# Banksylel/Restrictive-Hierarchical-Semantic-Segmentation

Measured on AMD Instinct MI355X. Metric: train images/sec (620x620, hier-HRNet-W48), higher is better.
Workload: dtype f32 (fp16x2 split on fp16 MFMA, 22-bit operands, fp32 accumulate; exact-fp32 MFMA on the small problems); 1 GPU; HRNet-W48 hierarchical (class_tree_tl.json), 620x620, batch 4 per GPU, train_epoch batch body (fwd L passes, prediction prep + metrics, CE+Dice+consistency, bwd, grad all-reduce, AdamW, metric vectors, one D2H readback of loss+metrics); global_batch=4, parallelism=dp1, launch=launch tape replay, rccl_ranks=1, level_passes=batched (one launch per layer for all L passes)

## Files before the change

restrictive-hierarchical-semantic-segmentation_amd/csrc/conv_sp.h:

```cpp
#pragma once
#include <type_traits>

typedef __bf16 bf16x8 __attribute__((ext_vector_type(8)));
typedef __bf16 bf16x2 __attribute__((ext_vector_type(2)));
typedef unsigned u32x4 __attribute__((ext_vector_type(4)));
typedef unsigned u32x2 __attribute__((ext_vector_type(2)));

__device__ __forceinline__ unsigned sp_pack_trunc(float lo, float hi) {
  return __builtin_amdgcn_perm(__float_as_uint(hi), __float_as_uint(lo), 0x07060302u);
}
__device__ __forceinline__ unsigned sp_pack_rne(float lo, float hi) {
  const bf16x2 v = {(__bf16)lo, (__bf16)hi};
  return __builtin_bit_cast(unsigned, v);
}
__device__ __forceinline__ float sp_trunc(float x) { return __uint_as_float(__float_as_uint(x) & 0xFFFF0000u); }

constexpr int sp_np(int ns) { return ns == 4 ? 2 : ns; }
constexpr int sp_products(int ns) { return ns == 1 ? 1 : ns == 3 ? 6 : 3; }
typedef _Float16 f16x8 __attribute__((ext_vector_type(8)));
typedef _Float16 f16x2 __attribute__((ext_vector_type(2)));

__device__ __forceinline__ void sp_pow2_scale(const float* absmax, float& scale, float& inv) {
  scale = inv = 1.f;
  if (!absmax) return;
// ... 1006 lines not shown
      u32x2 pc[sp_np(NS)];
      sp_split4<NS>(rp[i], pc, xscale);
      int f = tid + 256 * i;
      if (f >= PG) f -= 256;
      const int pix = f / (CS * 4), rem = f - pix * (CS * 4);
      const int c = rem >> 2, q = rem & 3;
      const int o = c * L::CHUNK + pix * 32 + ((q ^ (2 * ((pix >> 3) & 1))) << 3);
#pragma unroll
      for (int s = 0; s < sp_np(NS); ++s) *reinterpret_cast<u32x2*>(lpatch + s * L::PPIECE + o) = pc[s];
    }
  };

  unsigned wrow[W_LOADS];
  int wst[W_LOADS];
#pragma unroll
  for (int i = 0; i < W_LOADS; ++i) {
    int f = tid + 256 * i;
    if (f >= WG) f -= 256;
    const int n = f >> 3, unit = (f >> 2) & 1, gq = f & 3;
    wrow[i] = ((unsigned)n * (unsigned)(p.T * p.K) + 4u * gq) * 4u;
    wst[i] = n * 64 + lds_slot(n, gq) * 16 + unit * 8;
  }
  const bool wunit1 = (tid >> 2) & 1;
  f32x4 rwt[2][W_LOADS];
  constexpr int W16 = NS == 4 ? L::WSTAGE / 16 : 0;
  static_assert(W16 <= 256 * W_LOADS, "a pre-split slab fits the register set of an fp32 one");
  const bool img = NS == 4 && p.wimg != nullptr;
  const __amdgpu_buffer_rsrc_t rwi = make_rsrc(reinterpret_cast<const float*>(p.wimg), (size_t)ntn * nks * NSLAB * L::WSTAGE);
  auto w_load = [&](int n0, int ks, int slab, int set) {
    if (img) {
      const unsigned base = (unsigned)(((n0 / BN) * nks + ks) * NSLAB + slab) * (unsigned)L::WSTAGE;
#pragma unroll
      for (int i = 0; i < W_LOADS; ++i) {
        const int f = tid + 256 * i;
        rwt[set][i] = buf_load4(rwi, f < W16 ? base + (unsigned)f * 16u : HRSEG_BUF_OOB, 0);
      }
      return;
    }
    const int uA = 2 * slab, uB = 2 * slab + 1;
    const int tA = uA / CS, cA = uA - tA * CS, tB = uB / CS, cB = uB - tB * CS;
    const unsigned col0 = (unsigned)(n0 * p.T * p.K + ks * CS * 16) * 4u;
    const unsigned sA = col0 + (unsigned)(tA * p.K + cA * 16) * 4u;
    const unsigned sB = (uB < NU) ? col0 + (unsigned)(tB * p.K + cB * 16) * 4u : HRSEG_BUF_OOB;
    const unsigned so = wunit1 ? sB : sA;
#pragma unroll
    for (int i = 0; i < W_LOADS; ++i) {
      const unsigned off = (so == HRSEG_BUF_OOB) ? HRSEG_BUF_OOB : wrow[i] + so;
      rwt[set][i] = buf_load4(rw, off, 0);
    }
  };
  auto w_store = [&](int wboff, int set) {
    unsigned char* base = lw + wboff;
    if (img) {
#pragma unroll
      for (int i = 0; i < W_LOADS; ++i) {
        const int f = tid + 256 * i;
        if (f < W16) *reinterpret_cast<f32x4*>(base + f * 16) = rwt[set][i];
      }
      return;
    }
#pragma unroll
    for (int i = 0; i < W_LOADS; ++i) {
      u32x2 pc[sp_np(NS)];
      sp_split4<NS>(rwt[set][i], pc, p.wscale);
#pragma unroll
      for (int s = 0; s < sp_np(NS); ++s) *reinterpret_cast<u32x2*>(base + s * L::WPIECE + wst[i]) = pc[s];
    }
  };

  const int foff = r16 * 64 + lds_slot(r16, g) * 16;
  const int prow0 = (wave * RPW) * PW + r16;
  const int pbase = prow0 * 32;

  auto read_frags = [&](int slab, int wboff, bf16x8 (&xf)[RPW][sp_np(NS)], bf16x8 (&wf)[WTN][sp_np(NS)]) {
    const int uA = 2 * slab, uB = 2 * slab + 1;
    const int tA = uA / CS, cA = uA - tA * CS;
    const int tB = (uB < NU) ? uB / CS : 0, cB = (uB < NU) ? uB - tB * CS : 0;
    const int dA = (FLIP ? 2 - tA / 3 : tA / 3) * PW + (FLIP ? 2 - tA % 3 : tA % 3);
    const int dB = (FLIP ? 2 - tB / 3 : tB / 3) * PW + (FLIP ? 2 - tB % 3 : tB % 3);
#pragma unroll
    for (int m = 0; m < RPW; ++m) {
      const int pa = prow0 + m * PW + dA, pb = prow0 + m * PW + dB;
      const int oa = cA * L::CHUNK + pbase + (m * PW + dA) * 32 + ((g ^ (2 * ((pa >> 3) & 1))) << 3);
      const int ob = cB * L::CHUNK + pbase + (m * PW + dB) * 32 + ((g ^ (2 * ((pb >> 3) & 1))) << 3);
#pragma unroll
      for (int q = 0; q < sp_np(NS); ++q) {
        const u32x2 lo = *reinterpret_cast<const u32x2*>(lpatch + q * L::PPIECE + oa);
        u32x2 hi = u32x2{0u, 0u};
        if (uB < NU) hi = *reinterpret_cast<const u32x2*>(lpatch + q * L::PPIECE + ob);
        xf[m][q] = __builtin_bit_cast(bf16x8, (u32x4){lo[0], lo[1], hi[0], hi[1]});
      }
    }
    const unsigned char* base = lw + wboff;
#pragma unroll
    for (int n = 0; n < WTN; ++n)
#pragma unroll
      for (int q = 0; q < sp_np(NS); ++q) wf[n][q] = *reinterpret_cast<const bf16x8*>(base + q * L::WPIECE + n * 1024 + foff);
  };

  f32x4 acc[WTN][RPW];
  auto zero_acc = [&]() {
#pragma unroll
    for (int n = 0; n < WTN; ++n)
#pragma unroll
      for (int m = 0; m < RPW; ++m) acc[n][m] = f32x4{0.f, 0.f, 0.f, 0.f};
  };
  auto store_tile = [&](const Geom& q) {
    f32x4 add[RPW][WTN];
#pragma unroll
    for (int n = 0; n < WTN; ++n) {
      f32x4 bv = f32x4{0.f, 0.f, 0.f, 0.f};
      if (p.bias) bv = *reinterpret_cast<const f32x4*>(p.bias + q.n0 + 16 * n + 4 * g);
#pragma unroll
      for (int m = 0; m < RPW; ++m) add[m][n] = bv;
    }
    if (p.accumulate) {
#pragma unroll
      for (int m = 0; m < RPW; ++m) {
        const int oy = q.y0 + wave * RPW + m, ox = q.x0 + r16;
        if (oy >= H || ox >= W) continue;
        const float* yrow = p.y + ((size_t)(q.b * H + oy) * W + ox) * p.ldy;
#pragma unroll
        for (int n = 0; n < WTN; ++n) add[m][n] += *reinterpret_cast<const f32x4*>(yrow + q.n0 + 16 * n + 4 * g);
      }
    }
    if (p.res) {
#pragma unroll
      for (int m = 0; m < RPW; ++m) {
        const int oy = q.y0 + wave * RPW + m, ox = q.x0 + r16;
        if (oy >= H || ox >= W) continue;
        const float* rrow = p.res + ((size_t)(q.b * H + oy) * W + ox) * p.ldr;
#pragma unroll
        for (int n = 0; n < WTN; ++n) add[m][n] += *reinterpret_cast<const f32x4*>(rrow + q.n0 + 16 * n + 4 * g);
      }
    }
#pragma unroll
    for (int m = 0; m < RPW; ++m) {
      const int oy = q.y0 + wave * RPW + m, ox = q.x0 + r16;
      if (oy >= H || ox >= W) continue;
      float* yrow = p.y + ((size_t)(q.b * H + oy) * W + ox) * p.ldy;
#pragma unroll
      for (int n = 0; n < WTN; ++n) {
        f32x4 v = acc[n][m];
        if (NS == 4) v *= oscale;
        v += add[m][n];
        if (p.relu) {
#pragma unroll
          for (int e = 0; e < 4; ++e) v[e] = fmaxf(v[e], 0.f);
        }
        *reinterpret_cast<f32x4*>(yrow + q.n0 + 16 * n + 4 * g) = v;
      }
    }
  };

  bf16x8 xfr[2][RPW][sp_np(NS)], wfr[2][WTN][sp_np(NS)];
  int t = first;
  Geom cur = tile_geom(t);
  patch_load(cur, 0);
  w_load(cur.n0, 0, 0, 0);
  w_load(cur.n0, 0, 1, 1);
  patch_store();
  w_store(0, 0);
  w_store(L::WSTAGE, 1);
  w_load(cur.n0, 0, 2, 0);
  __syncthreads();
  read_frags(0, 0, xfr[0], wfr[0]);
  zero_acc();
  int wb = 0;
  for (;;) {
    bool have_next = false;
    for (int ks = 0; ks < nks; ++ks) {
      const bool last_ks = ks + 1 == nks;
      const int nt = last_ks ? t + stride : t;
      const int nks_ = last_ks ? 0 : ks + 1;
      have_next = nt < end;
      Geom nxt = cur;
      if (last_ks && have_next) nxt = tile_geom(nt);
#pragma unroll
      for (int s = 0; s < NSLAB; ++s) {
        const int wb1 = (wb == 2 * L::WSTAGE) ? 0 : wb + L::WSTAGE;
        const int wb2 = (wb1 == 2 * L::WSTAGE) ? 0 : wb1 + L::WSTAGE;
        if (s + 3 < NSLAB) w_load(cur.n0, ks, s + 3, (s + 1) & 1);
        else if (have_next) w_load(nxt.n0, nks_, s + 3 - NSLAB, (s + 1) & 1);
        if (s == NSLAB - 3 && have_next) patch_load(nxt, nks_);
        if (s + 1 < NSLAB) read_frags(s + 1, wb1, xfr[(s + 1) & 1], wfr[(s + 1) & 1]);
#pragma unroll
        for (int pr = 0; pr < sp_nprod(NS); ++pr)
#pragma unroll
          for (int n = 0; n < WTN; ++n)
#pragma unroll
            for (int m = 0; m < RPW; ++m) acc[n][m] = sp_mma_p<NS>(pr, wfr[s & 1][n], xfr[s & 1][m], acc[n][m]);
        if (s + 2 < NSLAB || have_next) w_store(wb2, s & 1);
        if (s == NSLAB - 1) {
          if (last_ks) { store_tile(cur); zero_acc(); }
          if (have_next) patch_store();
        }
        __syncthreads();
        if (s == NSLAB - 1 && have_next) read_frags(0, wb1, xfr[0], wfr[0]);
        wb = wb1;
      }
      if (last_ks) cur = nxt;
    }
    if (!have_next) break;
    t += stride;
  }
}

constexpr int sp_patch_min_waves(int ns, int wtn, int cs) { return (ns == 3 || (wtn == 6 && cs == 4)) ? 1 : 2; }
template <int NS, int TH, int WTN, int CS, int FLIP>
__global__ __launch_bounds__(256) __attribute__((amdgpu_waves_per_eu(sp_patch_min_waves(NS, WTN, CS), 2)))
void igemm_patch_sp_kernel(IgemmArgs p, int ntotal) {
  __shared__ __attribute__((aligned(16))) unsigned char lds[SpPatchLds<NS, TH, WTN, CS>::BYTES];
  const int chunk = (ntotal + gridDim.x - 1) / gridDim.x;
  const int first = blockIdx.x * chunk;
  igemm_patch_sp_body<NS, TH, WTN, CS, FLIP>(p, lds, first, 1, min(first + chunk, ntotal));
}

template <int NS, int TH, int WTN, int CS>
struct SpPatchWsLds {
  using P = SpPatchLds<NS, TH, WTN, CS>;
  static constexpr int STAT_MAXN = 1024;
  static constexpr int STAT = 2 * STAT_MAXN * 8;
  static constexpr int BYTES = 2 * P::PATCH + 3 * P::WSTAGE + STAT;
  static constexpr int NSLAB = (9 * CS + 1) / 2;
};

template <int NS, int WTN, int CS>
__device__ __forceinline__ void sp_weight_image_body(const float* __restrict__ w, unsigned char* __restrict__ img, int K,
                                                     float wscale, int blk) {
  using L = SpPatchLds<NS, 8, WTN, CS>;
  constexpr int BN = 16 * WTN, WG = BN * 8, NU = 9 * CS, NSLAB = (NU + 1) / 2;
  const int nks = K / (16 * CS);
  const int slab = blk % NSLAB;
  const int ks = (blk / NSLAB) % nks;
  const int nt = blk / (NSLAB * nks);
  unsigned char* dst = img + (size_t)blk * L::WSTAGE;
  for (int f = threadIdx.x; f < WG; f += 256) {
    const int n = f >> 3, unit = (f >> 2) & 1, gq = f & 3;
    const int u = 2 * slab + unit;
    f32x4 v = {0.f, 0.f, 0.f, 0.f};
    if (u < NU) {
      const int t = u / CS, c = u - t * CS;
      v = *reinterpret_cast<const f32x4*>(w + ((size_t)(nt * BN + n) * 9 + t) * K + ks * CS * 16 + c * 16 + 4 * gq);
    }
    u32x2 pc[sp_np(NS)];
    sp_split4<NS>(v, pc, wscale);
    const int o = n * 64 + lds_slot(n, gq) * 16 + unit * 8;
#pragma unroll
    for (int q = 0; q < sp_np(NS); ++q) *reinterpret_cast<u32x2*>(dst + q * L::WPIECE + o) = pc[q];
  }
}
struct WeightImageGroup {
  int n;
  int ns;
  int blk_end[MAXG];
  int kind[MAXG];
  int K[MAXG];
  float wscale[MAXG];
  const float* w[MAXG];
  unsigned char* img[MAXG];
};
struct WeightImageTabEntry {
  const float* w;
  unsigned char* img;
  int K, kind, ns, blk_end;
  float wscale;
  int pad;
};
#ifdef HRSEG_TU_WS
__global__ __launch_bounds__(256) void sp_weight_image_table_kernel(const WeightImageTabEntry* __restrict__ tab, int n) {
  int lo = 0, hi = n - 1;
  while (lo < hi) {
    const int mid = (lo + hi) >> 1;
    if ((int)blockIdx.x >= tab[mid].blk_end) lo = mid + 1; else hi = mid;
  }
  const WeightImageTabEntry e = tab[lo];
  const int blk = blockIdx.x - (lo ? tab[lo - 1].blk_end : 0);
  if (e.ns == 1) {
    if (e.kind == 2) sp_weight_image_body<1, 6, 3>(e.w, e.img, e.K, e.wscale, blk);
    else if (e.kind == 3) sp_weight_image_body<1, 4, 4>(e.w, e.img, e.K, e.wscale, blk);
    else sp_weight_image_body<1, 3, 3>(e.w, e.img, e.K, e.wscale, blk);
    return;
  }
  if (e.kind == 2) sp_weight_image_body<4, 6, 3>(e.w, e.img, e.K, e.wscale, blk);
  else if (e.kind == 3) sp_weight_image_body<4, 4, 4>(e.w, e.img, e.K, e.wscale, blk);
  else sp_weight_image_body<4, 3, 3>(e.w, e.img, e.K, e.wscale, blk);
}
__global__ __launch_bounds__(256) void sp_weight_image_kernel(WeightImageGroup g) {
  int gi = 0;
  while (gi + 1 < g.n && (int)blockIdx.x >= g.blk_end[gi]) ++gi;
  const int blk = blockIdx.x - (gi ? g.blk_end[gi - 1] : 0);
  const int kind = g.kind[gi];
  if (g.ns == 1) {
    if (kind == 2) sp_weight_image_body<1, 6, 3>(g.w[gi], g.img[gi], g.K[gi], g.wscale[gi], blk);
    else if (kind == 3) sp_weight_image_body<1, 4, 4>(g.w[gi], g.img[gi], g.K[gi], g.wscale[gi], blk);
    else sp_weight_image_body<1, 3, 3>(g.w[gi], g.img[gi], g.K[gi], g.wscale[gi], blk);
    return;
  }
  if (kind == 2) sp_weight_image_body<4, 6, 3>(g.w[gi], g.img[gi], g.K[gi], g.wscale[gi], blk);
  else if (kind == 3) sp_weight_image_body<4, 4, 4>(g.w[gi], g.img[gi], g.K[gi], g.wscale[gi], blk);
  else sp_weight_image_body<4, 3, 3>(g.w[gi], g.img[gi], g.K[gi], g.wscale[gi], blk);
}
#endif

__device__ __forceinline__ float sp_row16_sum(float v) {
  v += __builtin_bit_cast(float, __builtin_amdgcn_update_dpp(0, __builtin_bit_cast(int, v), 0x111, 0xf, 0xf, true));
  v += __builtin_bit_cast(float, __builtin_amdgcn_update_dpp(0, __builtin_bit_cast(int, v), 0x112, 0xf, 0xf, true));
  v += __builtin_bit_cast(float, __builtin_amdgcn_update_dpp(0, __builtin_bit_cast(int, v), 0x114, 0xf, 0xf, true));
  v += __builtin_bit_cast(float, __builtin_amdgcn_update_dpp(0, __builtin_bit_cast(int, v), 0x118, 0xf, 0xf, true));
  return v;
}

__device__ __forceinline__ void sp_wait_vm(f32x4& r, int n) {
  switch (n) {
#define HRSEG_VM(N) case N: asm volatile("s_waitcnt vmcnt(" #N ")" : "+v"(r)); break;
    HRSEG_VM(0) HRSEG_VM(1) HRSEG_VM(2) HRSEG_VM(3) HRSEG_VM(4) HRSEG_VM(5) HRSEG_VM(6) HRSEG_VM(7) HRSEG_VM(8) HRSEG_VM(9)
    HRSEG_VM(10) HRSEG_VM(11) HRSEG_VM(12) HRSEG_VM(13) HRSEG_VM(14) HRSEG_VM(15) HRSEG_VM(16) HRSEG_VM(17) HRSEG_VM(18) HRSEG_VM(19)
    HRSEG_VM(20) HRSEG_VM(21) HRSEG_VM(22) HRSEG_VM(23) HRSEG_VM(24) HRSEG_VM(25) HRSEG_VM(26) HRSEG_VM(27) HRSEG_VM(28) HRSEG_VM(29)
    HRSEG_VM(30) HRSEG_VM(31) HRSEG_VM(32) HRSEG_VM(33) HRSEG_VM(34) HRSEG_VM(35) HRSEG_VM(36) HRSEG_VM(37) HRSEG_VM(38) HRSEG_VM(39)
    HRSEG_VM(40) HRSEG_VM(41) HRSEG_VM(42) HRSEG_VM(43) HRSEG_VM(44) HRSEG_VM(45) HRSEG_VM(46) HRSEG_VM(47) HRSEG_VM(48)
#undef HRSEG_VM
    default: asm volatile("s_waitcnt vmcnt(0)" : "+v"(r)); break;
  }
}

template <int NS, int TH, int WTN, int CS, int FLIP>
__device__ __forceinline__ void igemm_patch_ws_body(const IgemmArgs& p, unsigned char* lds, const int first, const int end,
                                                    const int block_row = 0) {
  static_assert(NS == 4 || NS == 1, "the wave-specialised body: fp16x2 (two pieces, three products) or bf16 (one piece, one product)");
  using L = SpPatchLds<NS, TH, WTN, CS>;
  constexpr int RPW = TH / 4, BN = 16 * WTN, PW = 18, PP = L::PP;
  constexpr int GPP = CS * 4, PR = 256 / GPP;
  constexpr int P_LOADS = (PP + PR - 1) / PR;
  constexpr int W16 = L::WSTAGE / 16, W_LOADS = (W16 + 255) / 256;
  constexpr int NU = 9 * CS, NSLAB = (NU + 1) / 2;
#ifndef HRSEG_WS_EXP
#define HRSEG_WS_EXP 0
#endif
  static_assert(NSLAB % 2 == 0, "register-set parity must restart with every K stage");
  unsigned char* lpatch = lds;
  unsigned char* lw = lds + 2 * L::PATCH;
  double* lstat = reinterpret_cast<double*>(lds + 2 * L::PATCH + 3 * L::WSTAGE);
  const int tid = threadIdx.x, lane = tid & 63, wave = tid >> 6;
  const bool consumer = __builtin_amdgcn_readfirstlane(wave) < 4;
  const int ptid = tid & 255;
  const int r16 = lane & 15, g = lane >> 4;
  const int H = p.Ho, W = p.Wo;
  const int cv_w1 = p.cv_w1, cv_nb = p.cv_w1 > 0 ? p.cv_nb : 1;
  const unsigned cv_magic = p.cv_w1 > 0 ? p.cv_magic : 0u;
  const int Wc = p.cv_w1 > 0 ? cv_nb * cv_w1 - 1 : W;
  const int tiles_x = (Wc + 15) >> 4, tiles_y = (H + TH - 1) / TH;
  const int ntn = p.N / BN;
  const int nks = p.K / (16 * CS);
  if (first >= end) return;
#ifndef HRSEG_WS_STAMP
#define HRSEG_WS_STAMP 0
#endif
#if HRSEG_WS_STAMP
  const bool stat = false;
  unsigned long long* const stamp_out = reinterpret_cast<unsigned long long*>(p.stat_partial);
  const bool stamping = stamp_out != nullptr && block_row == 0 && (wave == 0 || wave == 4);
  int stamp_j = 0;
  auto stamped_barrier = [&]() {
    unsigned long long t0, t1;
    asm volatile("s_memtime %0" : "=s"(t0));
    __builtin_amdgcn_s_barrier();
    asm volatile("s_memtime %0\n\ts_waitcnt lgkmcnt(0)" : "=s"(t1));
    if (stamping && stamp_j < 1024 && lane == 0) {
      unsigned long long* o = stamp_out + ((wave >> 2) * 1024 + stamp_j) * 2;
      o[0] = t0;
      o[1] = t1;
    }
    ++stamp_j;
  };
#else
  const bool stat = p.stat_partial != nullptr;
  auto stamped_barrier = [&]() { __builtin_amdgcn_s_barrier(); };
#endif
  if (stat)
    for (int i = tid; i < 2 * p.N; i += 512) lstat[i] = 0.0;

  struct Geom { int b, y0, x0, nt; };
  auto tile_geom = [&](int t) {
    Geom q;
    q.nt = t % ntn;
    int mt = t / ntn;
    const int tx = mt % tiles_x;
    mt /= tiles_x;
    const int ty = mt % tiles_y;
    q.b = mt / tiles_y;
    q.y0 = ty * TH; q.x0 = tx * 16;
    return q;
  };
  auto tile_next = [&](Geom& q) {
    if (++q.nt < ntn) return;
    q.nt = 0;
    q.x0 += 16;
    if (q.x0 < tiles_x * 16) return;
    q.x0 = 0;
    q.y0 += TH;
    if (q.y0 < tiles_y * TH) return;
    q.y0 = 0;
    ++q.b;
  };

  if (consumer) {
    float xscale, xinv;
    sp_pow2_scale(p.xmax, xscale, xinv);
    const float oscale = xinv * p.wscale_inv;
    const int foff = r16 * 64 + lds_slot(r16, g) * 16;
    const int prow0 = (wave * RPW) * PW + r16;
    const int pbase = prow0 * 32;
    constexpr int NP = sp_np(NS);
    constexpr int UNITS = RPW * NP + WTN * NP;
    constexpr int MM = WTN * RPW * sp_nprod(NS);
    int xbase[16];
#pragma unroll
    for (int j = 0; j < 16; ++j) xbase[j] = pbase + ((g ^ (2 * (((prow0 + j) >> 3) & 1))) << 3);
    auto xbase_flip = [&](int to_buf) {
#pragma unroll
      for (int j = 0; j < 16; ++j) xbase[j] += to_buf ? L::PATCH : -L::PATCH;
    };
    auto read_unit = [&](int slab, int wboff, int r, bf16x8 (&xf)[RPW][NP], bf16x8 (&wf)[WTN][NP]) {
      if (r < RPW * NP) {
        const int m = r / NP, q = r % NP;
        const int uA = 2 * slab, uB = 2 * slab + 1;
        const int tA = uA / CS, cA = uA - tA * CS;
        const int tB = (uB < NU) ? uB / CS : 0, cB = (uB < NU) ? uB - tB * CS : 0;
        const int dA = (FLIP ? 2 - tA / 3 : tA / 3) * PW + (FLIP ? 2 - tA % 3 : tA % 3);
        const int dB = (FLIP ? 2 - tB / 3 : tB / 3) * PW + (FLIP ? 2 - tB % 3 : tB % 3);
        const unsigned char* pb = lpatch + q * L::PPIECE;
        const int ca = m * PW + dA, cb = m * PW + dB;
        const u32x2 lo = *reinterpret_cast<const u32x2*>(pb + xbase[ca & 15] + (cA * L::CHUNK + ca * 32));
        u32x2 hi = u32x2{0u, 0u};
        if (uB < NU) hi = *reinterpret_cast<const u32x2*>(pb + xbase[cb & 15] + (cB * L::CHUNK + cb * 32));
        xf[m][q] = __builtin_bit_cast(bf16x8, (u32x4){lo[0], lo[1], hi[0], hi[1]});
      } else {
        const int i = r - RPW * NP, n = i / NP, q = i % NP;
        wf[n][q] = *reinterpret_cast<const bf16x8*>(lw + wboff + q * L::WPIECE + n * 1024 + foff);
      }
    };
    f32x4 acc[WTN][RPW];
    auto zero_acc = [&]() {
#pragma unroll
      for (int n = 0; n < WTN; ++n)
#pragma unroll
        for (int m = 0; m < RPW; ++m) acc[n][m] = f32x4{0.f, 0.f, 0.f, 0.f};
    };
    constexpr bool PF = WTN * RPW <= 8;
    constexpr int S_PF = NSLAB > 10 ? NSLAB - 10 : 0;
    f32x4 add[RPW][WTN];
    auto pin_i = [](int v) { return __builtin_amdgcn_readfirstlane(v); };
    auto pin_p = [](const void* ptr) {
      const unsigned long long a = (unsigned long long)ptr;
      const unsigned lo = (unsigned)__builtin_amdgcn_readfirstlane((int)(unsigned)(a & 0xffffffffull));
      const unsigned hi = (unsigned)__builtin_amdgcn_readfirstlane((int)(unsigned)(a >> 32));
      return (unsigned long long)lo | ((unsigned long long)hi << 32);
    };
    float* const e_y = reinterpret_cast<float*>(pin_p(p.y));
    const float* const e_bias = reinterpret_cast<const float*>(pin_p(p.bias));
    const float* const e_res = reinterpret_cast<const float*>(pin_p(p.res));
    const int e_ldy = pin_i(p.ldy), e_ldr = pin_i(p.ldr), e_acc = pin_i(p.accumulate), e_relu = pin_i(p.relu);
    const int e_early = pin_i(p.epi_early), e_stat = pin_i(stat ? 1 : 0), e_N = pin_i(p.N);
    constexpr bool SREG = PF;
    const int e_sreg = pin_i((stat && ntn == 1) ? 1 : 0);
    f32x4 rs1[SREG ? WTN : 1], rs2[SREG ? WTN : 1];
#pragma unroll
    for (int n = 0; n < (SREG ? WTN : 1); ++n) rs1[n] = rs2[n] = f32x4{0.f, 0.f, 0.f, 0.f};
    const unsigned ldy4 = (unsigned)e_ldy * 4u, ldr4 = (unsigned)e_ldr * 4u;
    const int wave_rows = pin_i(wave * RPW);
    const unsigned g16 = (unsigned)g * 16u;
    auto tile_offsets = [&](const Geom& q, unsigned ld4, unsigned (&off)[RPW]) {
      const int cxo = q.x0 + r16;
      const int obc = (int)__umulhi((unsigned)cxo, cv_magic);
      const int ox = cxo - obc * cv_w1;
      const bool ook = !(HRSEG_WS_EXP & 32) & (ox < W) & (obc < cv_nb);
      const int oy0 = q.y0 + wave_rows;
      const unsigned base = (unsigned)((obc * H + oy0) * W + ox) * ld4 + (unsigned)(q.nt * BN) * 4u + g16;
      const unsigned rowstep = (unsigned)W * ld4;
#pragma unroll
      for (int m = 0; m < RPW; ++m) off[m] = (ook & (oy0 + m < H)) ? base + (unsigned)m * rowstep : HRSEG_BUF_OOB;
    };
    const int e_nothing = pin_i((!p.bias && !p.accumulate && !p.res) ? 1 : 0);
    auto fetch_add = [&](const Geom& q) {
      if (e_nothing) {
#pragma unroll
        for (int m = 0; m < RPW; ++m)
#pragma unroll
          for (int n = 0; n < WTN; ++n) add[m][n] = f32x4{0.f, 0.f, 0.f, 0.f};
        return;
      }
#pragma unroll
      for (int n = 0; n < WTN; ++n) {
        f32x4 bv = f32x4{0.f, 0.f, 0.f, 0.f};
        if (e_bias) bv = *reinterpret_cast<const f32x4*>(e_bias + q.nt * BN + 16 * n + 4 * g);
#pragma unroll
        for (int m = 0; m < RPW; ++m) add[m][n] = bv;
      }
      if (e_acc) {
        const __amdgpu_buffer_rsrc_t ry = make_rsrc(e_y + (size_t)q.b * H * W * e_ldy, (size_t)cv_nb * H * W * ldy4);
        unsigned off[RPW];
        tile_offsets(q, ldy4, off);
#pragma unroll
        for (int m = 0; m < RPW; ++m)
#pragma unroll
          for (int n = 0; n < WTN; ++n) add[m][n] += buf_load4(ry, off[m], 64 * n);
      }
      if (e_res) {
        const __amdgpu_buffer_rsrc_t rr = make_rsrc(e_res + (size_t)q.b * H * W * e_ldr, (size_t)cv_nb * H * W * ldr4);
        unsigned off[RPW];
        tile_offsets(q, ldr4, off);
#pragma unroll
        for (int m = 0; m < RPW; ++m)
#pragma unroll
          for (int n = 0; n < WTN; ++n) add[m][n] += buf_load4(rr, off[m], 64 * n);
      }
    };
    auto store_acc_as = [&](const Geom& q, auto plain_tag) {
      constexpr bool PLAIN = decltype(plain_tag)::value;
      const __amdgpu_buffer_rsrc_t ry = make_rsrc(e_y + (size_t)q.b * H * W * e_ldy, (size_t)cv_nb * H * W * ldy4);
      unsigned off[RPW];
      tile_offsets(q, ldy4, off);
      if (e_stat) {
#pragma unroll
        for (int n = 0; n < WTN; ++n) {
          f32x4 s1 = {0.f, 0.f, 0.f, 0.f}, s2 = {0.f, 0.f, 0.f, 0.f};
#pragma unroll
          for (int m = 0; m < RPW; ++m) {
            const bool ok = off[m] != HRSEG_BUF_OOB;
            const f32x4 v = PLAIN ? acc[n][m] * oscale : acc[n][m] * oscale + add[m][n];
#pragma unroll
            for (int e = 0; e < 4; ++e) {
              const float ve = ok ? v[e] : 0.f;
              s1[e] += ve;
              s2[e] += ve * ve;
            }
          }
          if (SREG && e_sreg) {
            rs1[n] += s1;
            rs2[n] += s2;
            continue;
          }
#pragma unroll
          for (int e = 0; e < 4; ++e) {
            s1[e] = sp_row16_sum(s1[e]);
            s2[e] = sp_row16_sum(s2[e]);
          }
          if (r16 == 15) {
            const int c0 = q.nt * BN + 16 * n + 4 * g;
#pragma unroll
            for (int e = 0; e < 4; ++e) {
              __hip_atomic_fetch_add(lstat + c0 + e, (double)s1[e], __ATOMIC_RELAXED, __HIP_MEMORY_SCOPE_WORKGROUP);
              __hip_atomic_fetch_add(lstat + e_N + c0 + e, (double)s2[e], __ATOMIC_RELAXED, __HIP_MEMORY_SCOPE_WORKGROUP);
            }
          }
        }
      }
#pragma unroll
      for (int m = 0; m < RPW; ++m) {
#pragma unroll
        for (int n = 0; n < WTN; ++n) {
          f32x4 v = PLAIN ? acc[n][m] * oscale : acc[n][m] * oscale + add[m][n];
          if (!PLAIN && e_relu) {
#pragma unroll
            for (int e = 0; e < 4; ++e) v[e] = fmaxf(v[e], 0.f);
          }
          buf_store4(ry, off[m], 64 * n, v);
        }
        __builtin_amdgcn_sched_barrier(0);
        asm volatile("s_nop 7" ::: "memory");
        __builtin_amdgcn_sched_barrier(0);
      }
    };
    auto store_acc = [&](const Geom& q) { store_acc_as(q, std::false_type{}); };
    bf16x8 xfr[2][RPW][NP], wfr[2][WTN][NP];
    Geom cur = tile_geom(first);
    __syncthreads();
#pragma unroll
    for (int r = 0; r < UNITS; ++r) read_unit(0, 0, r, xfr[0], wfr[0]);
    zero_acc();
    int wb = 0, pb = 0;
    for (int t = first;; ++t) {
      bool have_next = false;
      for (int ks = 0; ks < nks; ++ks) {
        const bool last_ks = ks + 1 == nks;
        have_next = (last_ks ? t + 1 : t) < end;
#pragma unroll
        for (int s = 0; s < NSLAB; ++s) {
          const int wb1 = (wb == 2 * L::WSTAGE) ? 0 : wb + L::WSTAGE;
          const int nslab = (s + 1 < NSLAB) ? s + 1 : 0;
          if (s + 1 == NSLAB) xbase_flip(pb ^ 1);
          int k = 0;
#pragma unroll
          for (int pr = 0; pr < sp_nprod(NS); ++pr) {
#pragma unroll
            for (int n = 0; n < WTN; ++n) {
#pragma unroll
              for (int m = 0; m < RPW; ++m) {
                if (NS == 4) {
                  const f16x8 wv = __builtin_bit_cast(f16x8, wfr[s & 1][n][pr == 0 ? NP - 1 : 0]);
                  const f16x8 xv = __builtin_bit_cast(f16x8, xfr[s & 1][m][pr == 1 ? NP - 1 : 0]);
#if HRSEG_WS_EXP & 1
                  asm volatile("" :: "v"(wv), "v"(xv));
#else
                  acc[n][m] = __builtin_amdgcn_mfma_f32_16x16x32_f16(wv, xv, acc[n][m], 0, 0, 0);
#endif
                } else {
                  acc[n][m] = __builtin_amdgcn_mfma_f32_16x16x32_bf16(wfr[s & 1][n][0], xfr[s & 1][m][0], acc[n][m], 0, 0, 0);
                }
#pragma unroll
                for (int r = k * UNITS / MM; r < (k + 1) * UNITS / MM; ++r)
                  read_unit(nslab, wb1, r, xfr[(s + 1) & 1], wfr[(s + 1) & 1]);
                __builtin_amdgcn_sched_barrier(0);
                ++k;
              }
            }
          }
#if HRSEG_WS_EXP & 16
          if (s == NSLAB - 1 && last_ks) {
            if (acc[0][0][0] == 1.2345f) store_acc(cur);
            zero_acc();
          }
#else
          if (PF && s == S_PF && last_ks && e_early) fetch_add(cur);
          if (s == NSLAB - 1 && last_ks) {
#if HRSEG_WS_STAMP
            unsigned long long e0, e1, e2, e3;
            asm volatile("s_memtime %0\n\ts_waitcnt lgkmcnt(0)" : "=s"(e0) :: "memory");
            if (!(PF && e_early)) fetch_add(cur);
            asm volatile("s_memtime %0\n\ts_waitcnt lgkmcnt(0)" : "=s"(e1) :: "memory");
            store_acc(cur);
            asm volatile("s_memtime %0\n\ts_waitcnt lgkmcnt(0)" : "=s"(e2) :: "memory");
            zero_acc();
            asm volatile("s_memtime %0\n\ts_waitcnt lgkmcnt(0)" : "=s"(e3) :: "memory");
            if (stamping && wave == 0 && lane == 0 && stamp_j < 1024) {
              unsigned long long* o = stamp_out + 4096 + stamp_j * 4;
              o[0] = e0; o[1] = e1; o[2] = e2; o[3] = e3;
            }
#else
            if (!(PF && e_early)) fetch_add(cur);
            store_acc(cur);
            zero_acc();
#endif
          }
#endif
          asm volatile("s_waitcnt lgkmcnt(0)" ::: "memory");
          stamped_barrier();
          wb = wb1;
        }
        pb ^= 1;
        if (last_ks) tile_next(cur);
      }
      if (!have_next) break;
    }
    if (SREG && e_sreg) {
#pragma unroll
      for (int n = 0; n < WTN; ++n) {
#pragma unroll
        for (int e = 0; e < 4; ++e) {
          const float a = sp_row16_sum(rs1[n][e]), b = sp_row16_sum(rs2[n][e]);
          if (r16 == 15) {
            __hip_atomic_fetch_add(lstat + 16 * n + 4 * g + e, (double)a, __ATOMIC_RELAXED, __HIP_MEMORY_SCOPE_WORKGROUP);
            __hip_atomic_fetch_add(lstat + e_N + 16 * n + 4 * g + e, (double)b, __ATOMIC_RELAXED, __HIP_MEMORY_SCOPE_WORKGROUP);
          }
        }
      }
    }
  } else {
    float xscale, xinv;
    sp_pow2_scale(p.xmax, xscale, xinv);
    const int per_tile = nks * NSLAB;
    auto rsrc_words = [](const void* base, size_t bytes) {
      const unsigned long long a = (unsigned long long)base;
      i32x4_t r;
      r[0] = (int)(unsigned)(a & 0xffffffffull);
      r[1] = (int)(unsigned)((a >> 32) & 0xffffull);
      r[2] = (int)(unsigned)(bytes > 0xFFFFFFFFull ? 0xFFFFFFFFull : bytes);
      r[3] = HRSEG_BUF_FLAGS;
      return r;
    };
    auto ld16 = [](f32x4& dst, const i32x4_t& rs, unsigned voff, unsigned soff) {
      asm volatile("buffer_load_dwordx4 %0, %1, %2, %3 offen" : "=&v"(dst) : "v"(voff), "s"(rs), "s"(soff) : "memory");
    };
    const i32x4_t rw = rsrc_words(p.wimg, (size_t)ntn * per_tile * L::WSTAGE);
    const int pix0 = ptid / GPP, prem = ptid - pix0 * GPP;
    const bool pwork = pix0 < PR;
    const int pst0 = (prem >> 2) * L::CHUNK, pq = prem & 3;
    const unsigned ldx4 = (unsigned)p.ldx * 4u;
    unsigned rel[P_LOADS];
    int lst[P_LOADS];
    int gpy[P_LOADS], gpx[P_LOADS];
#pragma unroll
    for (int i = 0; i < P_LOADS; ++i) {
      const int pix = pix0 + PR * i;
      const int py = (pix * 3641) >> 16, px = pix - py * PW;
      const bool ex = pwork & (pix < PP);
      rel[i] = ex ? (unsigned)(py * W + px) * ldx4 + (unsigned)prem * 16u : HRSEG_BUF_OOB;
      lst[i] = ex ? pst0 + pix * 32 + ((pq ^ (2 * ((pix >> 3) & 1))) << 3) : PP * 32 + (lane & 15) * 8;
      gpy[i] = ex ? py : 0x40000000;
      gpx[i] = px;
    }
    static_assert(L::CHUNK - PP * 32 >= 128 + 8, "the padding of a chunk image takes the stores of granules that do not exist");
    unsigned wv[W_LOADS];
#pragma unroll
    for (int i = 0; i < W_LOADS; ++i) wv[i] = (ptid + 256 * i < W16) ? (unsigned)(ptid + 256 * i) * 16u : 0x80000000u;
    const bool wlast = __builtin_amdgcn_readfirstlane((int)((wave - 4) * 64 + 256 * (W_LOADS - 1) < W16)) != 0;
    const int wl0 = (int)(lw - lds) + ptid * 16;
    const int exp_nosplit = p.exp_nosplit | p.x_presplit;
    struct Stage { unsigned tb, tb0, delta; int y0m1, x0m1, xlo, xspan, xb; bool fast, second; };
    const unsigned hw = (unsigned)(H * W);
    auto stage_scalars = [&](const Geom& q) {
      Stage z;
      const int x0m1 = q.x0 - 1;
      z.y0m1 = q.y0 - 1;
      z.x0m1 = x0m1;
      z.xlo = x0m1 < 0 ? 1 : 0;
      if (cv_w1 > 0) {
        const int bc0 = x0m1 < 0 ? 0 : (int)__umulhi((unsigned)x0m1, cv_magic);
        z.xb = (bc0 + 1) * cv_w1 - x0m1;
        z.second = bc0 + 1 < cv_nb;
        z.tb0 = ((unsigned)((bc0 * H + z.y0m1) * W + x0m1 - bc0 * cv_w1)) * ldx4;
        z.delta = (hw - (unsigned)cv_w1) * ldx4;
        z.fast = false;
        if (bc0 >= cv_nb) z.xb = z.xlo + 1;
      } else {
        z.xb = W - x0m1 + 1;
        z.second = false;
        z.tb0 = (unsigned)(z.y0m1 * W + x0m1) * ldx4;
        z.delta = 0u;
        z.fast = (q.y0 >= 1) & (q.y0 + TH + 1 <= H) & (q.x0 >= 1) & (q.x0 + 17 <= W);
      }
      z.xspan = z.xb - 1 - z.xlo;
      z.tb = z.tb0;
      return z;
    };
    const bool cv_narrow = cv_w1 > 0 && cv_w1 < 18;
    auto patch_voff = [&](const Stage& z, int i) -> unsigned {
      if (cv_narrow) {
        const int iy = gpy[i] + z.y0m1, cx = gpx[i] + z.x0m1;
        const int bc = (int)__umulhi((unsigned)cx, cv_magic);
        const int ix = cx - bc * cv_w1;
        const bool ok = ((unsigned)iy < (unsigned)H) & (cx >= 0) & (ix < W) & (bc < cv_nb);
        return ok ? (unsigned)((bc * H + iy) * W + ix) * ldx4 + (unsigned)prem * 16u : HRSEG_BUF_OOB;
      }
      const bool oky = (unsigned)(gpy[i] + z.y0m1) < (unsigned)H;
      const bool ok1 = (unsigned)(gpx[i] - z.xlo) < (unsigned)z.xspan;
      const bool ok2 = z.second & (gpx[i] >= z.xb);
      const unsigned off = rel[i] + z.tb0 + (ok2 ? z.delta : 0u);
      return (oky & (ok1 | ok2)) ? off : HRSEG_BUF_OOB;
    };
    auto patch_store1 = [&](const f32x4& v, int i, int pboff) {
      u32x2 pc[sp_np(NS)];
      if (exp_nosplit) {
        const u32x4 raw = __builtin_bit_cast(u32x4, v);
#pragma unroll
        for (int s = 0; s < sp_np(NS); ++s) pc[s] = u32x2{raw[(2 * s) & 3], raw[(2 * s + 1) & 3]};
      } else {
        sp_split4<NS>(v, pc, xscale);
      }
      const int o = pboff + lst[i];
#pragma unroll
      for (int s = 0; s < sp_np(NS); ++s) *reinterpret_cast<u32x2*>(lpatch + s * L::PPIECE + o) = pc[s];
    };
    auto image_rsrc = [&](int b) { return rsrc_words(p.x + (size_t)b * H * W * p.ldx, (size_t)cv_nb * H * W * p.ldx * 4); };
    auto stage_woff = [&](int nt, int ks) { return (unsigned)((nt * nks + ks) * NSLAB) * (unsigned)L::WSTAGE; };
    constexpr int DW = 2;
    constexpr int GPL = (P_LOADS + NSLAB - 6) / (NSLAB - 5);
    constexpr int DP = NSLAB - 1 - (P_LOADS + GPL - 1) / GPL;
    static_assert(DP >= 4 && (P_LOADS + GPL - 1) / GPL <= NSLAB - DW, "patch schedule");
    f32x4 rw4[DW][W_LOADS], pg[P_LOADS];
    Geom cur = tile_geom(first);
    unsigned woff_cur = stage_woff(cur.nt, 0);
    {
      f32x4 v[P_LOADS];
      const i32x4_t rx0 = image_rsrc(cur.b);
      const Stage z0 = stage_scalars(cur);
#pragma unroll
      for (int i = 0; i < P_LOADS; ++i) ld16(v[i], rx0, patch_voff(z0, i), 0u);
      f32x4 w01[2][W_LOADS];
#pragma unroll
      for (int d = 0; d < 2; ++d)
#pragma unroll
        for (int i = 0; i < W_LOADS; ++i) ld16(w01[d][i], rw, wv[i] + woff_cur + (unsigned)(d * L::WSTAGE), 0u);
#pragma unroll
      for (int i = 0; i < P_LOADS; ++i) asm volatile("s_waitcnt vmcnt(0)" : "+v"(v[i]));
#pragma unroll
      for (int i = 0; i < P_LOADS; ++i) patch_store1(v[i], i, 0);
#pragma unroll
      for (int i = 0; i < W_LOADS; ++i) asm volatile("s_waitcnt vmcnt(0)" : "+v"(w01[0][i]), "+v"(w01[1][i]));
#pragma unroll
      for (int d = 0; d < 2; ++d)
#pragma unroll
        for (int i = 0; i < W_LOADS; ++i)
          if (i + 1 < W_LOADS || wlast) *reinterpret_cast<f32x4*>(lds + wl0 + d * L::WSTAGE + i * 4096) = w01[d][i];
    }
    int n_t = first, n_ks = 0;
    Geom nxt = cur;
    i32x4_t rxn = image_rsrc(cur.b);
    bool have_next = false;
    unsigned woff_nxt = 0u;
    auto advance = [&]() {
      if (++n_ks == nks) {
        n_ks = 0;
        ++n_t;
        const int b = nxt.b;
        tile_next(nxt);
        if (nxt.b != b) rxn = image_rsrc(nxt.b);
      }
      have_next = n_t < end;
      woff_nxt = stage_woff(nxt.nt, n_ks);
    };
    advance();
    auto slab_woff = [&](int k) { return k < NSLAB ? woff_cur + (unsigned)(k * L::WSTAGE) : woff_nxt + (unsigned)((k - NSLAB) * L::WSTAGE); };
    static_assert(2 + 2 * DW <= NSLAB, "weight look-ahead stays within the next stage");
#pragma unroll
    for (int d = 0; d < DW; ++d)
#pragma unroll
      for (int i = 0; i < W_LOADS; ++i) ld16(rw4[(d + 2) % DW][i], rw, wv[i] + slab_woff(d + 2), 0u);
    __syncthreads();
    int wb2 = 2 * L::WSTAGE;
    int pboff = 0;
    auto nl = [](int s) { s = ((s % NSLAB) + NSLAB) % NSLAB; const int r = P_LOADS - s * GPL; return r < 0 ? 0 : (r > GPL ? GPL : r); };
    const int nstages = (end - first) * nks;
    int q = 0;
    do {
      const Stage z = stage_scalars(nxt);
      const i32x4_t rx = have_next ? rxn : rsrc_words(p.x, 0);
      const unsigned soff = z.tb + (unsigned)(n_ks * CS * 64);
      const unsigned ksoff = (unsigned)(n_ks * CS * 64);
#pragma unroll
      for (int s = 0; s < NSLAB; ++s) {
        {
          int yw = nl(s - DW);
#pragma unroll
          for (int k = s - DW + 1; k < s; ++k) yw += W_LOADS + nl(k);
          f32x4 (&wset)[W_LOADS] = rw4[s % DW];
#pragma unroll
          for (int i = 0; i < W_LOADS; ++i) sp_wait_vm(wset[i], yw);
          const int a = wl0 + wb2;
#pragma unroll
          for (int i = 0; i < W_LOADS; ++i)
            if (!(HRSEG_WS_EXP & 8) && (i + 1 < W_LOADS || wlast)) *reinterpret_cast<f32x4*>(lds + a + i * 4096) = wset[i];
          const unsigned wo = slab_woff(s + 2 + DW);
#pragma unroll
          for (int i = 0; i < W_LOADS; ++i) ld16(wset[i], rw, (HRSEG_WS_EXP & 2) ? HRSEG_BUF_OOB : wv[i], wo);
        }
        if (s >= DP && nl(s - DP) > 0) {
          int yp = W_LOADS;
#pragma unroll
          for (int k = s - DP + 1; k < s; ++k) yp += W_LOADS + nl(k);
#pragma unroll
          for (int e = 0; e < GPL; ++e)
            if (e < nl(s - DP)) sp_wait_vm(pg[(s - DP) * GPL + e], yp + nl(s - DP) - 1 - e);
          if (have_next) {
#pragma unroll
            for (int e = 0; e < GPL; ++e)
              if (e < nl(s - DP)) patch_store1(pg[(s - DP) * GPL + e], (s - DP) * GPL + e, L::PATCH - pboff);
          }
        }
#pragma unroll
        for (int e = 0; e < GPL; ++e) {
          if (e < nl(s)) {
            const int i = s * GPL + e;
            if (HRSEG_WS_EXP & 4) ld16(pg[i], rx, HRSEG_BUF_OOB, 0u);
            else if (z.fast) ld16(pg[i], rx, rel[i], soff);
            else ld16(pg[i], rx, patch_voff(z, i), ksoff);
          }
        }
        asm volatile("s_waitcnt lgkmcnt(0)" ::: "memory");
        stamped_barrier();
        wb2 = (wb2 == 2 * L::WSTAGE) ? 0 : wb2 + L::WSTAGE;
      }
      pboff = L::PATCH - pboff;
      woff_cur = woff_nxt;
      advance();
    } while (++q < nstages);
    asm volatile("s_waitcnt vmcnt(0)" ::: "memory");
  }
  if (stat) {
    asm volatile("s_waitcnt lgkmcnt(0)" ::: "memory");
    __builtin_amdgcn_s_barrier();
    double* row = p.stat_partial + (size_t)block_row * 2 * p.N;
    for (int i = tid; i < 2 * p.N; i += 512) row[i] = lstat[i];
  }
}

template <int NS, int TH, int WTN, int CS, int FLIP>
__global__ __launch_bounds__(512) void igemm_patch_ws_kernel(IgemmArgs p, int ntotal) {
  __shared__ __attribute__((aligned(16))) unsigned char lds[SpPatchWsLds<NS, TH, WTN, CS>::BYTES];
  const int chunk = (ntotal + gridDim.x - 1) / gridDim.x;
  const int first = blockIdx.x * chunk;
  igemm_patch_ws_body<NS, TH, WTN, CS, FLIP>(p, lds, first, min(first + chunk, ntotal), blockIdx.x);
}

template <int NS, int FLIP>
__global__ __launch_bounds__(512) void igemm_patch_ws_group_kernel(IgemmGroup grp) {
  static_assert(SpPatchWsLds<NS, 16, 3, 3>::BYTES >= SpPatchWsLds<NS, 8, 4, 4>::BYTES &&
                SpPatchWsLds<NS, 16, 3, 3>::BYTES >= SpPatchWsLds<NS, 8, 6, 3>::BYTES, "LDS of the largest variant");
  __shared__ __attribute__((aligned(16))) unsigned char lds[SpPatchWsLds<NS, 16, 3, 3>::BYTES];
  int gi = 0;
  while (gi + 1 < grp.n && (int)blockIdx.x >= grp.blk_end[gi]) ++gi;
  const int local = blockIdx.x - (gi ? grp.blk_end[gi - 1] : 0);
  const int nblk = grp.tiles[gi], ntotal = grp.ksplit[gi];
  const int chunk = (ntotal + nblk - 1) / nblk;
  const int first = local * chunk, end = min(first + chunk, ntotal);
  const int kind = grp.kind[gi];
  if (kind == 1) igemm_patch_ws_body<NS, 8, 3, 3, FLIP>(grp.a[gi], lds, first, end, local);
  else if (kind == 2) igemm_patch_ws_body<NS, 8, 6, 3, FLIP>(grp.a[gi], lds, first, end, local);
  else if (kind == 3) igemm_patch_ws_body<NS, 8, 4, 4, FLIP>(grp.a[gi], lds, first, end, local);
  else igemm_patch_ws_body<NS, 16, 3, 3, FLIP>(grp.a[gi], lds, first, end, local);
}

template <int NS, int WTM, int WTN, int CS, int FLIP>
__global__ __launch_bounds__(256) __attribute__((amdgpu_waves_per_eu(sp_patch_min_waves(NS, WTN, CS), 2)))
void igemm_sp_pgroup_kernel(IgemmGroup grp) {
  constexpr int A = SpPatchLds<NS, 8, WTN, CS>::BYTES, B = SpLds<NS, WTN>::BYTES;
  __shared__ __attribute__((aligned(16))) unsigned char lds[A > B ? A : B];
  int gi = 0;
  while (gi + 1 < grp.n && (int)blockIdx.x >= grp.blk_end[gi]) ++gi;
  const int local = blockIdx.x - (gi ? grp.blk_end[gi - 1] : 0);
  const int tiles = grp.tiles[gi];
  if (grp.kind[gi]) igemm_patch_sp_body<NS, 8, WTN, CS, FLIP>(grp.a[gi], lds, local, 1 << 29, tiles);
  else igemm_sp_body<NS, WTM, WTN>(grp.a[gi], lds, local % tiles, tiles, local / tiles, grp.ksplit[gi]);
}

template <int NS, int TNK>
struct SpWgrad9Lds {
  static constexpr int S = sp_row_stride(16 * TNK);
  static constexpr int DYPIX = 64, XPIX = 6 * 18;
  static constexpr int PIECE = (DYPIX + XPIX) * S;
  static constexpr int BYTES = sp_np(NS) * PIECE;
};

struct Wgrad9Args {
  const float* x; const float* dy; float* ws;
  const float* dymax;
  int ldx, lddy, B, H, W, Cin, Cout;
  int tiles_x, tiles_y, ntiles, nchunks, per;
  int exp_nosplit;
  int x_presplit;
};

template <int NS, int TNK>
__device__ __forceinline__ void wgrad9_sp_body(const Wgrad9Args& p, unsigned char* lds, const int pair, const int chunk) {
  using L = SpWgrad9Lds<NS, TNK>;
  constexpr int S = L::S, PIECE = L::PIECE, XBASE = L::DYPIX * S;
  constexpr int GPP = TNK * 4;
  constexpr int NT = 192, PR = NT / GPP;
  constexpr int DY_LOADS = (L::DYPIX + PR - 1) / PR, X_LOADS = (L::XPIX + PR - 1) / PR, LOADS = DY_LOADS + X_LOADS;
  const int tid = threadIdx.x, lane = tid & 63, kh = tid >> 6;
  const int g = lane >> 4, li = lane & 15;
  const int nkt = p.Cin / (16 * TNK);
  const int ct = pair / nkt, kt = pair - ct * nkt;
  const int n0 = ct * 16 * TNK, k0 = kt * 16 * TNK;
  const int t_lo = chunk * p.per, t_hi = min(t_lo + p.per, p.ntiles);
  float dyscale, dyinv;
  sp_pow2_scale(p.dymax, dyscale, dyinv);
// ... 209 lines not shown
```

Before: 91.01 images/s.

## Defer conv tile epilogue into next tile's first slab, interleaved with MFMAs

Instead of scaling, storing and accumulating statistics for a finished output tile in a serial block after the last K-slab, the persistent conv kernel now folds the accumulator into the prefetched add buffer and spreads the ReLU/store/statistics pieces across the MFMA issue slots of the next tile's first slab. The last tile's epilogue is flushed after the loop. This aims to hide epilogue latency behind matrix-core work. In exchange it adds register pressure (eoff, extra rsrc, a live prev geometry), couples the early fetch_add ordering to S_PF>0, and makes the schedule more complex.

```diff
diff --git a/restrictive-hierarchical-semantic-segmentation_amd/csrc/conv_sp.h b/restrictive-hierarchical-semantic-segmentation_amd/csrc/conv_sp.h
--- a/restrictive-hierarchical-semantic-segmentation_amd/csrc/conv_sp.h
+++ b/restrictive-hierarchical-semantic-segmentation_amd/csrc/conv_sp.h
@@ -1332,6 +1332,11 @@
   else sp_weight_image_body<4, 3, 3>(g.w[gi], g.img[gi], g.K[gi], g.wscale[gi], blk);
 }
 #endif
+
+template <class F, int... I>
+__device__ __forceinline__ void sp_static_for(std::integer_sequence<int, I...>, F&& f) {
+  (f(std::integral_constant<int, I>{}), ...);
+}
 
 __device__ __forceinline__ float sp_row16_sum(float v) {
   v += __builtin_bit_cast(float, __builtin_amdgcn_update_dpp(0, __builtin_bit_cast(int, v), 0x111, 0xf, 0xf, true));
@@ -1603,6 +1608,72 @@
       }
     };
     auto store_acc = [&](const Geom& q) { store_acc_as(q, std::false_type{}); };
+    constexpr bool DEFER = !(HRSEG_WS_EXP & 16);
+    static_assert(!PF || S_PF > 0, "the early fetch_add of tile t+1 comes after tile t's deferred epilogue");
+    constexpr int EPN = 4 + RPW;
+    constexpr int EP = WTN * EPN;
+    constexpr int EPS = 2 * WTN * RPW;
+    auto ep_slot = [](int i) {
+      const int even = RPW - 1 + i * (EPS - RPW + 1) / EP, ready = (i / EPN + 1) * RPW - 1;
+      const int s = even > ready ? even : ready;
+      return s < MM - 1 ? s : MM - 1;
+    };
+    auto ep_first = [&](int k) {
+      int i = 0;
+      while (i < EP && ep_slot(i) < k) ++i;
+      return i;
+    };
+    Geom prev;
+    bool ep_live = false;
+    unsigned eoff[RPW];
+    __amdgpu_buffer_rsrc_t ery = make_rsrc(e_y, 0);
+    auto ep_scale = [&](int n, int m) __attribute__((always_inline)) {
+      if (n == 0 && m == 0) {
+        ery = make_rsrc(e_y + (size_t)prev.b * H * W * e_ldy, ep_live ? (size_t)cv_nb * H * W * ldy4 : 0);
+        tile_offsets(prev, ldy4, eoff);
+      }
+      add[m][n] = acc[n][m] * oscale + add[m][n];
+      acc[n][m] = f32x4{0.f, 0.f, 0.f, 0.f};
+    };
+    auto ep_piece = [&](int i) __attribute__((always_inline)) {
+      const int n = i / EPN, j = i % EPN;
+      if (j < 4) {
+        if (!(e_stat && ep_live)) return;
+        float s1 = 0.f, s2 = 0.f;
+#pragma unroll
+        for (int m = 0; m < RPW; ++m) {
+          const bool ok = eoff[m] != HRSEG_BUF_OOB;
+          const float ve = ok ? add[m][n][j] : 0.f;
+          s1 += ve;
+          s2 += ve * ve;
+        }
+        if constexpr (SREG) {
+          if (e_sreg) {
+            rs1[n][j] += s1;
+            rs2[n][j] += s2;
+            return;
+          }
+        }
+        s1 = sp_row16_sum(s1);
+        s2 = sp_row16_sum(s2);
+        if (r16 == 15) {
+          const int c = prev.nt * BN + 16 * n + 4 * g + j;
+          __hip_atomic_fetch_add(lstat + c, (double)s1, __ATOMIC_RELAXED, __HIP_MEMORY_SCOPE_WORKGROUP);
+          __hip_atomic_fetch_add(lstat + e_N + c, (double)s2, __ATOMIC_RELAXED, __HIP_MEMORY_SCOPE_WORKGROUP);
+        }
+        return;
+      }
+      const int m = j - 4;
+      f32x4 v = add[m][n];
+      if (e_relu) {
+#pragma unroll
+        for (int e = 0; e < 4; ++e) v[e] = fmaxf(v[e], 0.f);
+      }
+      buf_store4(ery, eoff[m], 64 * n, v);
+      __builtin_amdgcn_sched_barrier(0);
+      asm volatile("s_nop 7" ::: "memory");
+      __builtin_amdgcn_sched_barrier(0);
+    };
     bf16x8 xfr[2][RPW][NP], wfr[2][WTN][NP];
     Geom cur = tile_geom(first);
     __syncthreads();
@@ -1610,79 +1681,83 @@
     for (int r = 0; r < UNITS; ++r) read_unit(0, 0, r, xfr[0], wfr[0]);
     zero_acc();
     int wb = 0, pb = 0;
+    auto slab = [&](auto s_c, auto ep_c, const bool last_ks) __attribute__((always_inline)) {
+      constexpr int s = decltype(s_c)::value;
+      constexpr bool ep = decltype(ep_c)::value;
+      const int wb1 = (wb == 2 * L::WSTAGE) ? 0 : wb + L::WSTAGE;
+      const int nslab = (s + 1 < NSLAB) ? s + 1 : 0;
+      if (s + 1 == NSLAB) xbase_flip(pb ^ 1);
+      int k = 0;
+#pragma unroll
+      for (int pr = 0; pr < sp_nprod(NS); ++pr) {
+#pragma unroll
+        for (int n = 0; n < WTN; ++n) {
+#pragma unroll
+          for (int m = 0; m < RPW; ++m) {
+            if (s == 0 && pr == 0 && ep) ep_scale(n, m);
+            if (NS == 4) {
+              const f16x8 wv = __builtin_bit_cast(f16x8, wfr[s & 1][n][pr == 0 ? NP - 1 : 0]);
+              const f16x8 xv = __builtin_bit_cast(f16x8, xfr[s & 1][m][pr == 1 ? NP - 1 : 0]);
+#if HRSEG_WS_EXP & 1
+              asm volatile("" :: "v"(wv), "v"(xv));
+#else
+              acc[n][m] = __builtin_amdgcn_mfma_f32_16x16x32_f16(wv, xv, acc[n][m], 0, 0, 0);
+#endif
+            } else {
+              acc[n][m] = __builtin_amdgcn_mfma_f32_16x16x32_bf16(wfr[s & 1][n][0], xfr[s & 1][m][0], acc[n][m], 0, 0, 0);
+            }
+#pragma unroll
+            for (int r = k * UNITS / MM; r < (k + 1) * UNITS / MM; ++r)
+              read_unit(nslab, wb1, r, xfr[(s + 1) & 1], wfr[(s + 1) & 1]);
+            if (s == 0 && ep) {
+              for (int i = ep_first(k); i < ep_first(k + 1); ++i) ep_piece(i);
+            }
+            __builtin_amdgcn_sched_barrier(0);
+            ++k;
+          }
+        }
+      }
+#if HRSEG_WS_EXP & 16
+      if (s == NSLAB - 1 && last_ks) {
+        if (acc[0][0][0] == 1.2345f) store_acc(cur);
+        zero_acc();
+      }
+#else
+      if (PF && s == S_PF && last_ks && e_early) fetch_add(cur);
+#endif
+      asm volatile("s_waitcnt lgkmcnt(0)" ::: "memory");
+      stamped_barrier();
+      wb = wb1;
+    };
+    auto stage = [&](auto ep_c, const int ks) __attribute__((always_inline)) {
+      sp_static_for(std::make_integer_sequence<int, NSLAB>{}, [&](auto s_c) __attribute__((always_inline)) {
+        slab(s_c, std::integral_constant<bool, decltype(ep_c)::value && decltype(s_c)::value == 0>{}, ks + 1 == nks);
+      });
+      pb ^= 1;
+    };
     for (int t = first;; ++t) {
-      bool have_next = false;
-      for (int ks = 0; ks < nks; ++ks) {
-        const bool last_ks = ks + 1 == nks;
-        have_next = (last_ks ? t + 1 : t) < end;
-#pragma unroll
-        for (int s = 0; s < NSLAB; ++s) {
-          const int wb1 = (wb == 2 * L::WSTAGE) ? 0 : wb + L::WSTAGE;
-          const int nslab = (s + 1 < NSLAB) ? s + 1 : 0;
-          if (s + 1 == NSLAB) xbase_flip(pb ^ 1);
-          int k = 0;
-#pragma unroll
-          for (int pr = 0; pr < sp_nprod(NS); ++pr) {
-#pragma unroll
-            for (int n = 0; n < WTN; ++n) {
-#pragma unroll
-              for (int m = 0; m < RPW; ++m) {
-                if (NS == 4) {
-                  const f16x8 wv = __builtin_bit_cast(f16x8, wfr[s & 1][n][pr == 0 ? NP - 1 : 0]);
-                  const f16x8 xv = __builtin_bit_cast(f16x8, xfr[s & 1][m][pr == 1 ? NP - 1 : 0]);
-#if HRSEG_WS_EXP & 1
-                  asm volatile("" :: "v"(wv), "v"(xv));
+      stage(std::integral_constant<bool, DEFER>{}, 0);
+      for (int ks = 1; ks < nks; ++ks) stage(std::false_type{}, ks);
+      if (DEFER) {
+#if HRSEG_WS_STAMP
+        unsigned long long e0, e1;
+        asm volatile("s_memtime %0\n\ts_waitcnt lgkmcnt(0)" : "=s"(e0) :: "memory");
+        if (!(PF && e_early)) fetch_add(cur);
+        asm volatile("s_memtime %0\n\ts_waitcnt lgkmcnt(0)" : "=s"(e1) :: "memory");
+        if (stamping && wave == 0 && lane == 0 && stamp_j < 1024) {
+          unsigned long long* o = stamp_out + 4096 + stamp_j * 4;
+          o[0] = e0; o[1] = e1; o[2] = e1; o[3] = e1;
+        }
 #else
-                  acc[n][m] = __builtin_amdgcn_mfma_f32_16x16x32_f16(wv, xv, acc[n][m], 0, 0, 0);
+        if (!(PF && e_early)) fetch_add(cur);
 #endif
-                } else {
-                  acc[n][m] = __builtin_amdgcn_mfma_f32_16x16x32_bf16(wfr[s & 1][n][0], xfr[s & 1][m][0], acc[n][m], 0, 0, 0);
-                }
-#pragma unroll
-                for (int r = k * UNITS / MM; r < (k + 1) * UNITS / MM; ++r)
-                  read_unit(nslab, wb1, r, xfr[(s + 1) & 1], wfr[(s + 1) & 1]);
-                __builtin_amdgcn_sched_barrier(0);
-                ++k;
-              }
-            }
-          }
-#if HRSEG_WS_EXP & 16
-          if (s == NSLAB - 1 && last_ks) {
-            if (acc[0][0][0] == 1.2345f) store_acc(cur);
-            zero_acc();
-          }
-#else
-          if (PF && s == S_PF && last_ks && e_early) fetch_add(cur);
-          if (s == NSLAB - 1 && last_ks) {
-#if HRSEG_WS_STAMP
-            unsigned long long e0, e1, e2, e3;
-            asm volatile("s_memtime %0\n\ts_waitcnt lgkmcnt(0)" : "=s"(e0) :: "memory");
-            if (!(PF && e_early)) fetch_add(cur);
-            asm volatile("s_memtime %0\n\ts_waitcnt lgkmcnt(0)" : "=s"(e1) :: "memory");
-            store_acc(cur);
-            asm volatile("s_memtime %0\n\ts_waitcnt lgkmcnt(0)" : "=s"(e2) :: "memory");
-            zero_acc();
-            asm volatile("s_memtime %0\n\ts_waitcnt lgkmcnt(0)" : "=s"(e3) :: "memory");
-            if (stamping && wave == 0 && lane == 0 && stamp_j < 1024) {
-              unsigned long long* o = stamp_out + 4096 + stamp_j * 4;
-              o[0] = e0; o[1] = e1; o[2] = e2; o[3] = e3;
-            }
-#else
-            if (!(PF && e_early)) fetch_add(cur);
-            store_acc(cur);
-            zero_acc();
-#endif
-          }
-#endif
-          asm volatile("s_waitcnt lgkmcnt(0)" ::: "memory");
-          stamped_barrier();
-          wb = wb1;
-        }
-        pb ^= 1;
-        if (last_ks) tile_next(cur);
-      }
-      if (!have_next) break;
-    }
+        prev = cur;
+        ep_live = true;
+      }
+      tile_next(cur);
+      if (t + 1 >= end) break;
+    }
+    if (DEFER) store_acc(prev);
     if (SREG && e_sreg) {
 #pragma unroll
       for (int n = 0; n < WTN; ++n) {
```

Result: no change. 90.85 images/s (median of 3 runs) (-0.2%).
